# robotseu/ORB_Line_SLAM

Hardware: AMD Instinct MI355X
Metric: stereo frames/s extract+match (ORB+LBD), KITTI 1242x375 (higher is better)
Workload: dtype u8; 1 GPU; C3: 1242x375 stereo, 2000 ORB + 500 LBD per image, extract + stereo point/line match + f2f LBD match + SearchByBoW vs the previous frame (synthetic k=10 L=6 vocabulary, ComputeBoW included); parallelism=frame-sharded x1, distinct_pairs=512, order=shuffled, scene=default

## Files before the change

### orb_line_slam_amd/csrc/bow_match.hip

```cpp
#include "olf_internal.hpp"
#include "device_math.hpp"
#include "search_math.hpp"
#include "../../include/orbline.h"

namespace olf {

constexpr int BM_TH_LOW = 50;

__global__ __launch_bounds__(256) void k_bow_descend_nodes(const uint4* __restrict__ slotDesc, const int* __restrict__ childOff, const int* __restrict__ slotNode,
                                                           const double* __restrict__ nodeWeight, const uint4* __restrict__ desc, const int* __restrict__ counts,
                                                           int cap, int img_stride, int nid_level, int* __restrict__ nodeOut)
{
    const int f = blockIdx.y, i = blockIdx.x * 256 + threadIdx.x;
    if (i >= cap) return;
    int nid = -1;
    if (i < counts[(size_t)f * img_stride]) {
        const uint4* d = desc + 2 * ((size_t)f * img_stride * cap + i);
        const uint4 f0 = d[0], f1 = d[1];
        int node = 0, level = 0;
        int b = childOff[0], e = childOff[1];
        while (e > b) {
            ++level;
            int best = b, bd = 257;
            for (int s = b; s < e; ++s) {
                const uint4 c0 = slotDesc[2 * (size_t)s], c1 = slotDesc[2 * (size_t)s + 1];
                const int dd = ham256(f0, f1, c0, c1);
                if (dd < bd) { bd = dd; best = s; }
            }
            node = slotNode[best];
            if (level == nid_level) nid = node;
            b = childOff[node]; e = childOff[node + 1];
        }
        if (!(nodeWeight[node] > 0)) nid = -1;
        else if (nid < 0) nid = 0;
    }
    nodeOut[(size_t)f * cap + i] = nid;
}

__global__ __launch_bounds__(256) void k_bow_sort_nodes(const int* __restrict__ nodeIn, int cap, int P, unsigned long long* __restrict__ sorted, int* __restrict__ mOut)
{
    extern __shared__ unsigned long long s_key[];
    __shared__ int s_m;
    const int f = blockIdx.x;
    if (threadIdx.x == 0) s_m = 0;
    __syncthreads();
    int mine = 0;
    for (int i = threadIdx.x; i < P; i += 256) {
        const int nd = i < cap ? nodeIn[(size_t)f * cap + i] : -1;
        s_key[i] = nd >= 0 ? ((unsigned long long)nd << 16) | (unsigned)i : ~0ull;
        mine += nd >= 0;
    }
    if (mine) atomicAdd(&s_m, mine);
    __syncthreads();
    for (int k = 2; k <= P; k <<= 1)
        for (int j = k >> 1; j > 0; j >>= 1) {
            for (int t = threadIdx.x; t < P / 2; t += 256) {
                const int lo = ((t & ~(j - 1)) << 1) | (t & (j - 1)), hi = lo | j;
                const bool up = (lo & k) == 0;
                const unsigned long long a = s_key[lo], b = s_key[hi];
                if ((a > b) == up) { s_key[lo] = b; s_key[hi] = a; }
            }
            __syncthreads();
        }
    for (int i = threadIdx.x; i < cap; i += 256) sorted[(size_t)f * cap + i] = s_key[i];
    if (threadIdx.x == 0) mOut[f] = s_m;
}

constexpr int BM_WAVES = 8;

template <int FORM>
__device__ __forceinline__ void bow_node_walk(const unsigned long long* __restrict__ SK, int kb, int ke, const unsigned long long* __restrict__ SF, int fb, int fe,
                                              const uint4* __restrict__ dK, const uint4* __restrict__ dF, const olf_keypoint* __restrict__ kK,
                                              const olf_keypoint* __restrict__ kF, const uint8_t* __restrict__ validK, const uint8_t* __restrict__ badK,
                                              float nnratio, int checkOri, int lane, int* row, uint8_t* taken, uint8_t* binOf, int* hist, int* n)
{
    for (int q = kb; q < ke; ++q) {
        const int iKF = (int)(SK[q] & 0xffffu);
        if (validK && !validK[iKF]) continue;
        if (badK && badK[iKF]) continue;
        const uint4 a0 = dK[2 * (size_t)iKF], a1 = dK[2 * (size_t)iKF + 1];
        int b1 = 256, bi = -1, b2 = 256;
        for (int c0 = fb; c0 < fe; c0 += 64) {
            const bool on = c0 + lane < fe;
            const int iF = on ? (int)(SF[c0 + lane] & 0xffffu) : 0;
            int d = 0x7fff;
            if (on && (FORM == OLF_BOW_KF_FRAME ? row[iF] < 0 : taken[iF] == 0)) {
                const uint4 x0 = dF[2 * (size_t)iF], x1 = dF[2 * (size_t)iF + 1];
                d = ham256(a0, a1, x0, x1);
            }
            const int key = wave_min_i32((d << 6) | lane);
            const int c1 = key >> 6, cl = key & 63;
            const int d2 = wave_min_i32(lane == cl ? 0x7fff : d);
            if (c1 < 0x7fff) {
                const int ci = __builtin_amdgcn_readlane(iF, cl);
                if (c1 < b1) { b2 = min(b1, min(d2, 256)); b1 = c1; bi = ci; }
                else b2 = min(b2, c1);
            }
        }
        if ((FORM == OLF_BOW_KF_FRAME ? b1 <= BM_TH_LOW : b1 < BM_TH_LOW) && static_cast<float>(b1) < nnratio * static_cast<float>(b2)) {
            if (lane == 0) {
                const int at = FORM == OLF_BOW_KF_FRAME ? bi : iKF;
                if (FORM == OLF_BOW_KF_FRAME) row[bi] = iKF;
                else { row[iKF] = bi; taken[bi] = 1; }
                if (checkOri) {
                    int bin = rot_bin(kK[iKF].angle, kF[bi].angle);
                    bin = min(max(bin, 0), HISTO_LENGTH - 1);
                    binOf[at] = (uint8_t)bin;
                    atomicAdd(&hist[bin], 1);
                }
                atomicAdd(n, 1);
            }
            __builtin_amdgcn_wave_barrier();
        }
    }
}

__global__ __launch_bounds__(64 * BM_WAVES) void k_search_by_bow(const unsigned long long* __restrict__ sortedAll, const int* __restrict__ mAll, const olf_keypoint* __restrict__ kps,
                                                       const uint4* __restrict__ desc, const int* __restrict__ counts, int cap, int img_stride,
                                                       const uint8_t* __restrict__ mpValid, const uint8_t* __restrict__ mpBad, float nnratio, int checkOri,
                                                       int* __restrict__ matches, int* __restrict__ nmatches)
{
    extern __shared__ int s_mem[];
    __shared__ int s_hist[HISTO_LENGTH], s_seg, s_n, s_keep[3];
    int* matched = s_mem;
    uint8_t* binOf = reinterpret_cast<uint8_t*>(s_mem + cap);
    const int p = blockIdx.x, lane = threadIdx.x & 63;
    const int fK = p, fF = p + 1;
    const unsigned long long* SK = sortedAll + (size_t)fK * cap;
    const unsigned long long* SF = sortedAll + (size_t)fF * cap;
    const int mK = mAll[fK], mF = mAll[fF], nF = counts[(size_t)fF * img_stride];
    const olf_keypoint* kK = kps + (size_t)fK * img_stride * cap;
    const olf_keypoint* kF = kps + (size_t)fF * img_stride * cap;
    const uint4* dK = desc + 2 * (size_t)fK * img_stride * cap;
    const uint4* dF = desc + 2 * (size_t)fF * img_stride * cap;
    for (int i = threadIdx.x; i < cap; i += 64 * BM_WAVES) { matched[i] = -1; binOf[i] = 0; }
    if (threadIdx.x < HISTO_LENGTH) s_hist[threadIdx.x] = 0;
    if (threadIdx.x == 0) { s_seg = 0; s_n = 0; }
    __syncthreads();
    for (;;) {
        int kb = 0, ke = 0;
        if (lane == 0) {
            for (;;) {
                kb = atomicAdd(&s_seg, 0);
                if (kb >= mK) { ke = kb; break; }
                const unsigned long long node = SK[kb] >> 16;
                ke = bm_lower_bound(SK, mK, (node + 1) << 16);
                if (atomicCAS(&s_seg, kb, ke) == kb) break;
            }
        }
        kb = __builtin_amdgcn_readfirstlane(kb); ke = __builtin_amdgcn_readfirstlane(ke);
        if (kb >= mK) break;
        const unsigned long long node = SK[kb] >> 16;
        const int fb = bm_lower_bound(SF, mF, node << 16), fe = bm_lower_bound(SF, mF, (node + 1) << 16);
        if (fe <= fb) continue;
        bow_node_walk<OLF_BOW_KF_FRAME>(SK, kb, ke, SF, fb, fe, dK, dF, kK, kF, mpValid ? mpValid + (size_t)fK * cap : nullptr,
                                        mpBad ? mpBad + (size_t)fK * cap : nullptr, nnratio, checkOri, lane, matched, nullptr, binOf, s_hist, &s_n);
    }
    __syncthreads();
    if (checkOri) {
        if (threadIdx.x == 0) {
            int ind1, ind2, ind3;
            three_maxima(s_hist, ind1, ind2, ind3);
            s_keep[0] = ind1; s_keep[1] = ind2; s_keep[2] = ind3;
        }
        __syncthreads();
        int dropped = 0;
        for (int i = threadIdx.x; i < nF; i += 64 * BM_WAVES)
            if (matched[i] >= 0) { const int b = binOf[i]; if (b != s_keep[0] && b != s_keep[1] && b != s_keep[2]) { matched[i] = -1; ++dropped; } }
        if (dropped) atomicSub(&s_n, dropped);
        __syncthreads();
    }
    for (int i = threadIdx.x; i < cap; i += 64 * BM_WAVES) matches[(size_t)p * cap + i] = i < nF ? matched[i] : -1;
    if (threadIdx.x == 0) nmatches[p] = s_n;
}

int launch_bow_feature_vectors(const uint8_t* slotDesc, const int* childOff, const int* slotNode, const double* nodeWeight, int nid_level, int n_frames,
                               int img_stride, int cap, const uint8_t* d_desc, const int* d_counts, int* d_nodes, unsigned long long* d_sorted, int* d_m,
                               hipStream_t s)
{
    int P = 64;
    while (P < cap) P <<= 1;
    hipLaunchKernelGGL(k_bow_descend_nodes, dim3((cap + 255) / 256, n_frames), dim3(256), 0, s, reinterpret_cast<const uint4*>(slotDesc), childOff, slotNode,
                       nodeWeight, reinterpret_cast<const uint4*>(d_desc), d_counts, cap, img_stride, nid_level, d_nodes);
    hipLaunchKernelGGL(k_bow_sort_nodes, dim3(n_frames), dim3(256), (size_t)P * 8, s, d_nodes, cap, P, d_sorted, d_m);
    OLF_HIP_CHECK(hipGetLastError());
    return OLF_OK;
}

int launch_search_by_bow_batch(const uint8_t* slotDesc, const int* childOff, const int* slotNode, const double* nodeWeight, int nid_level, int n_frames,
                               int img_stride, int cap, const olf_keypoint* d_kps, const uint8_t* d_desc, const int* d_counts, const uint8_t* d_mp_valid,
                               const uint8_t* d_mp_bad, float nnratio, int check_ori, int* d_nodes, unsigned long long* d_sorted, int* d_m, int* d_matches,
                               int* d_nmatches, hipStream_t s)
{
    if (n_frames < 2) return OLF_OK;
    if (cap > 4096) { set_error("olf_search_by_bow_batch_dev: more than 4096 features per frame (the per-frame node sort runs in 32 KB of LDS)"); return OLF_ERR_CAPACITY; }
    OLF_TRY(launch_bow_feature_vectors(slotDesc, childOff, slotNode, nodeWeight, nid_level, n_frames, img_stride, cap, d_desc, d_counts, d_nodes, d_sorted, d_m, s));
    hipLaunchKernelGGL(k_search_by_bow, dim3(n_frames - 1), dim3(64 * BM_WAVES), (size_t)cap * 4 + ((cap + 3) & ~3), s, d_sorted, d_m, d_kps,
                       reinterpret_cast<const uint4*>(d_desc), d_counts, cap, img_stride, d_mp_valid, d_mp_bad, nnratio, check_ori, d_matches, d_nmatches);
    OLF_HIP_CHECK(hipGetLastError());
    return OLF_OK;
}

struct BowPairsArgs {
    const olf_keypoint* kps; const uint4* desc; const int* counts; const uint8_t* mpValid; const uint8_t* mpBad;
    const int* pairs;
    int cap, img_stride, n_frames, checkOri;
    float nnratio;
};

template <int FORM>
__global__ __launch_bounds__(64 * BM_WAVES) void k_search_by_bow_pairs(BowPairsArgs A, const unsigned long long* __restrict__ sortedAll, const int* __restrict__ mAll,
                                                                       int* __restrict__ status, int* __restrict__ matches, int* __restrict__ nmatches)
{
    extern __shared__ int s_mem[];
    __shared__ int s_hist[HISTO_LENGTH], s_seg, s_n, s_keep[3];
    const int cap = A.cap, p = blockIdx.x, tid = threadIdx.x, lane = tid & 63;
    int* row = s_mem;
    uint8_t* binOf = reinterpret_cast<uint8_t*>(s_mem + cap);
    uint8_t* taken = binOf + ((cap + 3) & ~3);
    const int f1 = A.pairs[2 * (size_t)p], f2 = A.pairs[2 * (size_t)p + 1];
    if (!pair_in_batch(f1, f2, A.n_frames)) {
        if (tid == 0) { nmatches[p] = -1; atomicOr(status, STATUS_PAIR); }
        return;
    }
    const size_t st = (size_t)A.img_stride;
    const unsigned long long* SK = sortedAll + (size_t)f1 * cap;
    const unsigned long long* SF = sortedAll + (size_t)f2 * cap;
    const int mK = mAll[f1], mF = mAll[f2];
    const int nRow = min(max(A.counts[(size_t)(FORM == OLF_BOW_KF_FRAME ? f2 : f1) * st], 0), cap);
    const olf_keypoint* kK = A.kps + (size_t)f1 * st * cap;
    const olf_keypoint* kF = A.kps + (size_t)f2 * st * cap;
    const uint4* dK = A.desc + 2 * (size_t)f1 * st * cap;
    const uint4* dF = A.desc + 2 * (size_t)f2 * st * cap;
    const uint8_t* validK = A.mpValid ? A.mpValid + (size_t)f1 * cap : nullptr;
    const uint8_t* badK = A.mpBad ? A.mpBad + (size_t)f1 * cap : nullptr;
    for (int i = tid; i < cap; i += 64 * BM_WAVES) {
        row[i] = -1; binOf[i] = 0;
        if (FORM == OLF_BOW_KF_KF) taken[i] = (A.mpValid && !A.mpValid[(size_t)f2 * cap + i]) || (A.mpBad && A.mpBad[(size_t)f2 * cap + i]) ? 1 : 0;
    }
    if (tid < HISTO_LENGTH) s_hist[tid] = 0;
    if (tid == 0) { s_seg = 0; s_n = 0; }
    __syncthreads();
    for (;;) {
        int kb = 0, ke = 0;
        if (lane == 0) {
            for (;;) {
                kb = atomicAdd(&s_seg, 0);
                if (kb >= mK) { ke = kb; break; }
                const unsigned long long node = SK[kb] >> 16;
                ke = bm_lower_bound(SK, mK, (node + 1) << 16);
                if (atomicCAS(&s_seg, kb, ke) == kb) break;
            }
        }
        kb = __builtin_amdgcn_readfirstlane(kb); ke = __builtin_amdgcn_readfirstlane(ke);
        if (kb >= mK) break;
        const unsigned long long node = SK[kb] >> 16;
        const int fb = bm_lower_bound(SF, mF, node << 16), fe = bm_lower_bound(SF, mF, (node + 1) << 16);
        if (fe <= fb) continue;
        bow_node_walk<FORM>(SK, kb, ke, SF, fb, fe, dK, dF, kK, kF, validK, badK, A.nnratio, A.checkOri, lane, row, taken, binOf, s_hist, &s_n);
    }
    __syncthreads();
    if (A.checkOri) {
        if (tid == 0) {
            int ind1, ind2, ind3;
            three_maxima(s_hist, ind1, ind2, ind3);
            s_keep[0] = ind1; s_keep[1] = ind2; s_keep[2] = ind3;
        }
        __syncthreads();
        int dropped = 0;
        for (int i = tid; i < nRow; i += 64 * BM_WAVES)
            if (row[i] >= 0) { const int b = binOf[i]; if (b != s_keep[0] && b != s_keep[1] && b != s_keep[2]) { row[i] = -1; ++dropped; } }
        if (dropped) atomicSub(&s_n, dropped);
        __syncthreads();
    }
    for (int i = tid; i < cap; i += 64 * BM_WAVES) matches[(size_t)p * cap + i] = row[i];
    if (tid == 0) nmatches[p] = s_n;
}

int launch_search_by_bow_pairs(const olf_track_batch& in, int n_frames, int cap, int n_pairs, const int* d_pairs, const uint8_t* d_mp_bad, int form, float nnratio,
                               int check_ori, const unsigned long long* d_sorted, const int* d_m, int* d_status, int* d_matches, int* d_nmatches, hipStream_t s)
{
    BowPairsArgs A;
    A.kps = in.kps; A.desc = reinterpret_cast<const uint4*>(in.desc); A.counts = in.counts; A.mpValid = in.mp_valid; A.mpBad = d_mp_bad;
    A.pairs = d_pairs; A.cap = cap; A.img_stride = in.img_stride; A.n_frames = n_frames; A.checkOri = check_ori; A.nnratio = nnratio;
    const size_t rowBytes = (size_t)cap * 4 + ((cap + 3) & ~3);
    if (form == OLF_BOW_KF_FRAME)
        hipLaunchKernelGGL(k_search_by_bow_pairs<OLF_BOW_KF_FRAME>, dim3(n_pairs), dim3(64 * BM_WAVES), rowBytes, s, A, d_sorted, d_m, d_status, d_matches, d_nmatches);
    else
        hipLaunchKernelGGL(k_search_by_bow_pairs<OLF_BOW_KF_KF>, dim3(n_pairs), dim3(64 * BM_WAVES), rowBytes + ((cap + 3) & ~3), s, A, d_sorted, d_m, d_status, d_matches,
                           d_nmatches);
    OLF_HIP_CHECK(hipGetLastError());
    return OLF_OK;
}

}
```

### orb_line_slam_amd/csrc/filters.hip

```cpp
#include "olf_internal.hpp"
#include <algorithm>

namespace olf {

constexpr int SF_TW = 128, SF_TH = 32;
constexpr int SF_INW = (SF_TW + 8) / 4;
constexpr int SF_INH = SF_TH + 6;

__device__ __forceinline__ int sf_reflect(int p, int n)
{
    if (p < 0) p = -p;
    if (p >= n) p = 2 * (n - 1) - p;
    return p;
}

__global__ __launch_bounds__(256) void k_sep7(const uint8_t* __restrict__ src, size_t srcImgStride, int srcPitch, uint8_t* __restrict__ dst,
                                              size_t dstImgStride, int dstPitch, int W, int H, Taps7 taps)
{
    __shared__ uint32_t s_in[SF_INH * SF_INW];
    constexpr int HS = (SF_INH + 1) / 2 + ((((SF_INH + 1) / 2) & 1) ? 0 : 1);
    __shared__ uint32_t s_h[SF_TW * HS];
    const int img = blockIdx.z, x0 = blockIdx.x * SF_TW, y0 = blockIdx.y * SF_TH;
    const uint8_t* s = src + (size_t)img * srcImgStride;
    const bool plain = x0 >= 4 && x0 + SF_TW + 4 <= W && y0 >= 3 && y0 + SF_TH + 3 <= H && ((srcPitch | (int)srcImgStride) & 3) == 0 &&
                       (reinterpret_cast<uintptr_t>(src) & 3) == 0;
    const uint8_t* tile = s + (ptrdiff_t)(y0 - 3) * srcPitch + (x0 - 4);
    for (int i = threadIdx.x; i < SF_INH * SF_INW; i += 256) {
        const int r = i / SF_INW, j = i - r * SF_INW;
        uint32_t v;
        if (plain) v = *reinterpret_cast<const uint32_t*>(tile + (size_t)r * srcPitch + 4 * j);
        else {
            const int gy = sf_reflect(min(y0 - 3 + r, H + 2), H);
            const int xw = x0 - 4 + 4 * j;
            const uint8_t* row = s + (size_t)gy * srcPitch;
            const uintptr_t addr = reinterpret_cast<uintptr_t>(row + xw);
            const int sh = (int)(addr & 3) * 8;
            if (xw >= 0 && (sh ? xw + 7 < W : xw + 3 < W)) {
                const uint32_t* p4 = reinterpret_cast<const uint32_t*>(row + xw - (int)(addr & 3));
                v = sh ? __funnelshift_r(p4[0], p4[1], sh) : p4[0];
            } else {
                v = 0;
#pragma unroll
                for (int b = 0; b < 4; ++b) v |= (uint32_t)row[sf_reflect(min(xw + b, W + 2), W)] << (8 * b);
            }
        }
        s_in[i] = v;
    }
    __syncthreads();
    const uint32_t tlo = (uint32_t)taps.t[0] | ((uint32_t)taps.t[1] << 8) | ((uint32_t)taps.t[2] << 16) | ((uint32_t)taps.t[3] << 24);
    const uint32_t thi = (uint32_t)taps.t[4] | ((uint32_t)taps.t[5] << 8) | ((uint32_t)taps.t[6] << 16);
    uint16_t* s_h16 = reinterpret_cast<uint16_t*>(s_h);
    for (int i = threadIdx.x; i < SF_INH * (SF_TW / 4); i += 256) {
        const int r = i / (SF_TW / 4), q = i - r * (SF_TW / 4);
        const uint32_t w0 = s_in[r * SF_INW + q], w1 = s_in[r * SF_INW + q + 1], w2 = s_in[r * SF_INW + q + 2];
        const uint32_t o0 = __builtin_amdgcn_udot4(__builtin_amdgcn_alignbyte(w2, w1, 1u), thi, __builtin_amdgcn_udot4(__builtin_amdgcn_alignbyte(w1, w0, 1u), tlo, 0u, false), false);
        const uint32_t o1 = __builtin_amdgcn_udot4(__builtin_amdgcn_alignbyte(w2, w1, 2u), thi, __builtin_amdgcn_udot4(__builtin_amdgcn_alignbyte(w1, w0, 2u), tlo, 0u, false), false);
        const uint32_t o2 = __builtin_amdgcn_udot4(__builtin_amdgcn_alignbyte(w2, w1, 3u), thi, __builtin_amdgcn_udot4(__builtin_amdgcn_alignbyte(w1, w0, 3u), tlo, 0u, false), false);
        const uint32_t o3 = __builtin_amdgcn_udot4(w2, thi, __builtin_amdgcn_udot4(w1, tlo, 0u, false), false);
        uint16_t* col = s_h16 + (size_t)(4 * q) * (2 * HS) + r;
        col[0] = (uint16_t)o0; col[2 * HS] = (uint16_t)o1; col[4 * HS] = (uint16_t)o2; col[6 * HS] = (uint16_t)o3;
    }
    __syncthreads();
    const int q = threadIdx.x & 31, ry0 = (threadIdx.x >> 5) * 4;
    const int gx = x0 + 4 * q;
    if (gx >= W) return;
    const uint32_t t01 = (uint32_t)taps.t[0] | ((uint32_t)taps.t[1] << 16), t23 = (uint32_t)taps.t[2] | ((uint32_t)taps.t[3] << 16);
    const uint32_t t45 = (uint32_t)taps.t[4] | ((uint32_t)taps.t[5] << 16), t6lo = (uint32_t)taps.t[6], t6hi = (uint32_t)taps.t[6] << 16;
    typedef unsigned short us2 __attribute__((ext_vector_type(2)));
    auto dot2 = [](uint32_t a, uint32_t b, uint32_t c) -> uint32_t {
        us2 va, vb;
        __builtin_memcpy(&va, &a, 4); __builtin_memcpy(&vb, &b, 4);
        return __builtin_amdgcn_udot2(va, vb, c, false);
    };
    uint32_t res[4][4];
#pragma unroll
    for (int c = 0; c < 4; ++c) {
        const uint32_t* hp = s_h + (size_t)(4 * q + c) * HS + (ry0 >> 1);
        const uint32_t D0 = hp[0], D1 = hp[1], D2 = hp[2], D3 = hp[3], D4 = hp[4];
        const uint32_t E0 = __builtin_amdgcn_alignbyte(D1, D0, 2u), E1 = __builtin_amdgcn_alignbyte(D2, D1, 2u);
        const uint32_t E2 = __builtin_amdgcn_alignbyte(D3, D2, 2u), E3 = __builtin_amdgcn_alignbyte(D4, D3, 2u);
        res[0][c] = dot2(D3, t6lo, dot2(D2, t45, dot2(D1, t23, dot2(D0, t01, 32768u))));
        res[1][c] = dot2(D3, t6hi, dot2(E2, t45, dot2(E1, t23, dot2(E0, t01, 32768u))));
        res[2][c] = dot2(D4, t6lo, dot2(D3, t45, dot2(D2, t23, dot2(D1, t01, 32768u))));
        res[3][c] = dot2(D4, t6hi, dot2(E3, t45, dot2(E2, t23, dot2(E1, t01, 32768u))));
    }
    uint8_t* d = dst + (size_t)img * dstImgStride;
#pragma unroll
    for (int rr = 0; rr < 4; ++rr) {
        const int gy = y0 + ry0 + rr;
        if (gy >= H) break;
        const uint32_t a0 = min(res[rr][0] >> 16, 255u), a1 = min(res[rr][1] >> 16, 255u), a2 = min(res[rr][2] >> 16, 255u), a3 = min(res[rr][3] >> 16, 255u);
        uint8_t* o = d + (size_t)gy * dstPitch + gx;
        if (gx + 3 < W && ((reinterpret_cast<uintptr_t>(o) & 3) == 0))
            *reinterpret_cast<uint32_t*>(o) = a0 | (a1 << 8) | (a2 << 16) | (a3 << 24);
        else {
            o[0] = (uint8_t)a0;
            if (gx + 1 < W) o[1] = (uint8_t)a1;
            if (gx + 2 < W) o[2] = (uint8_t)a2;
            if (gx + 3 < W) o[3] = (uint8_t)a3;
        }
    }
}

constexpr int SS_ROWS = 16;
constexpr int SS_BROWS = 8;

__device__ __forceinline__ int ss_reflect(int p, int n) { p = p < 0 ? -p : p; return p >= n ? 2 * (n - 1) - p : p; }

template <bool BORDER, int ROWS>
__device__ __forceinline__ void sep7_strip_body(const int t, const uint8_t* __restrict__ src, size_t srcImgStride, int srcPitch, uint8_t* __restrict__ dst,
                                                size_t dstImgStride, int dstPitch, int W, int H, const Taps7& taps, int nsx, int nsy)
{
    const int nb = BORDER ? 1 + ((W + 3) / 4 - (nsx + 1)) : nsx;
    if (t >= nb * nsy) return;
    const int sy = t / nb, si = t - sy * nb;
    const int sx = BORDER ? (si == 0 ? 0 : nsx + si) : si + 1;
    const int x0 = 4 * sx, y0 = sy * ROWS;
    const uint8_t* s = src + (size_t)blockIdx.y * srcImgStride + (x0 - 4);
    uint8_t* d = dst + (size_t)blockIdx.y * dstImgStride + x0;
    const uint32_t tlo = (uint32_t)taps.t[0] | ((uint32_t)taps.t[1] << 8) | ((uint32_t)taps.t[2] << 16) | ((uint32_t)taps.t[3] << 24);
    const uint32_t thi = (uint32_t)taps.t[4] | ((uint32_t)taps.t[5] << 8) | ((uint32_t)taps.t[6] << 16);
    const uint32_t t01 = (uint32_t)taps.t[0] | ((uint32_t)taps.t[1] << 16), t23 = (uint32_t)taps.t[2] | ((uint32_t)taps.t[3] << 16);
    const uint32_t t45 = (uint32_t)taps.t[4] | ((uint32_t)taps.t[5] << 16), t6lo = (uint32_t)taps.t[6], t6hi = (uint32_t)taps.t[6] << 16;
    typedef unsigned short us2 __attribute__((ext_vector_type(2)));
    auto dot2 = [](uint32_t a, uint32_t b, uint32_t c) -> uint32_t {
        us2 va, vb;
        __builtin_memcpy(&va, &a, 4); __builtin_memcpy(&vb, &b, 4);
        return __builtin_amdgcn_udot2(va, vb, c, false);
    };
    struct Raw { uint32_t w[3]; };
    auto load_row = [&](int y) -> Raw {
        Raw r;
        const uint8_t* row = s + (size_t)ss_reflect(min(y, H + 2), H) * srcPitch;
        if (!BORDER) __builtin_memcpy(r.w, row, 12);
        else {
#pragma unroll
            for (int k = 0; k < 3; ++k) {
                uint32_t v = 0;
#pragma unroll
                for (int b = 0; b < 4; ++b) {
                    const int x = x0 - 4 + 4 * k + b;
                    v |= (uint32_t)row[ss_reflect(min(x, W + 2), W) - (x0 - 4)] << (8 * b);
                }
                r.w[k] = v;
            }
        }
        return r;
    };
    auto hrow = [&](const Raw& r, uint32_t* o) {
        const uint32_t* w = r.w;
        o[0] = __builtin_amdgcn_udot4(__builtin_amdgcn_alignbyte(w[2], w[1], 1u), thi, __builtin_amdgcn_udot4(__builtin_amdgcn_alignbyte(w[1], w[0], 1u), tlo, 0u, false), false);
        o[1] = __builtin_amdgcn_udot4(__builtin_amdgcn_alignbyte(w[2], w[1], 2u), thi, __builtin_amdgcn_udot4(__builtin_amdgcn_alignbyte(w[1], w[0], 2u), tlo, 0u, false), false);
        o[2] = __builtin_amdgcn_udot4(__builtin_amdgcn_alignbyte(w[2], w[1], 3u), thi, __builtin_amdgcn_udot4(__builtin_amdgcn_alignbyte(w[1], w[0], 3u), tlo, 0u, false), false);
        o[3] = __builtin_amdgcn_udot4(w[2], thi, __builtin_amdgcn_udot4(w[1], tlo, 0u, false), false);
    };
    auto pair = [&](const Raw& ra, const Raw& rb, uint32_t* Pj) {
        uint32_t a[4], b[4];
        hrow(ra, a); hrow(rb, b);
#pragma unroll
        for (int c = 0; c < 4; ++c) Pj[c] = a[c] | (b[c] << 16);
    };
    uint32_t P[ROWS / 2 + 3][4];
    Raw nx[4];
    {
        Raw r0 = load_row(y0 - 3), r1 = load_row(y0 - 2), r2 = load_row(y0 - 1), r3 = load_row(y0), r4 = load_row(y0 + 1), r5 = load_row(y0 + 2);
#pragma unroll
        for (int k = 0; k < 4; ++k) nx[k] = load_row(y0 + 3 + k);
        pair(r0, r1, P[0]); pair(r2, r3, P[1]); pair(r4, r5, P[2]);
    }
#pragma unroll
    for (int g = 0; g < ROWS / 4; ++g) {
        const Raw c0 = nx[0], c1 = nx[1], c2 = nx[2], c3 = nx[3];
        if (g + 1 < ROWS / 4) {
#pragma unroll
            for (int k = 0; k < 4; ++k) nx[k] = load_row(y0 + 4 * (g + 1) + 3 + k);
            __builtin_amdgcn_sched_barrier(0);
        }
        pair(c0, c1, P[2 * g + 3]); pair(c2, c3, P[2 * g + 4]);
        uint32_t res[4][4];
#pragma unroll
        for (int c = 0; c < 4; ++c) {
            const uint32_t D0 = P[2 * g][c], D1 = P[2 * g + 1][c], D2 = P[2 * g + 2][c], D3 = P[2 * g + 3][c], D4 = P[2 * g + 4][c];
            const uint32_t E0 = __builtin_amdgcn_alignbyte(D1, D0, 2u), E1 = __builtin_amdgcn_alignbyte(D2, D1, 2u);
            const uint32_t E2 = __builtin_amdgcn_alignbyte(D3, D2, 2u), E3 = __builtin_amdgcn_alignbyte(D4, D3, 2u);
            res[0][c] = dot2(D3, t6lo, dot2(D2, t45, dot2(D1, t23, dot2(D0, t01, 32768u))));
            res[1][c] = dot2(D3, t6hi, dot2(E2, t45, dot2(E1, t23, dot2(E0, t01, 32768u))));
            res[2][c] = dot2(D4, t6lo, dot2(D3, t45, dot2(D2, t23, dot2(D1, t01, 32768u))));
            res[3][c] = dot2(D4, t6hi, dot2(E3, t45, dot2(E2, t23, dot2(E1, t01, 32768u))));
        }
#pragma unroll
        for (int rr = 0; rr < 4; ++rr) {
            const int gy = y0 + 4 * g + rr;
            if (gy < H) {
                const uint32_t a0 = min(res[rr][0] >> 16, 255u), a1 = min(res[rr][1] >> 16, 255u), a2 = min(res[rr][2] >> 16, 255u), a3 = min(res[rr][3] >> 16, 255u);
                const uint32_t v = a0 | (a1 << 8) | (a2 << 16) | (a3 << 24);
                if (!BORDER) __builtin_memcpy(d + (size_t)gy * dstPitch, &v, 4);
                else {
#pragma unroll
                    for (int b = 0; b < 4; ++b) if (x0 + b < W) d[(size_t)gy * dstPitch + b] = (uint8_t)(v >> (8 * b));
                }
            }
        }
    }
}

template <bool BORDER>
__global__ __launch_bounds__(256) void k_sep7_strip(const uint8_t* __restrict__ src, size_t srcImgStride, int srcPitch, uint8_t* __restrict__ dst,
                                                    size_t dstImgStride, int dstPitch, int W, int H, Taps7 taps, int nsx, int nsy)
{
    sep7_strip_body<BORDER, BORDER ? SS_BROWS : SS_ROWS>(blockIdx.x * 256 + threadIdx.x, src, srcImgStride, srcPitch, dst, dstImgStride, dstPitch, W, H, taps, nsx, nsy);
}

int launch_sep7(const uint8_t* src, size_t srcImgStride, int srcPitch, uint8_t* dst, size_t dstImgStride, int dstPitch, int W, int H,
                const int* taps7, int n_images, hipStream_t s)
{
    Taps7 t;
    for (int i = 0; i < 7; ++i) t.t[i] = taps7[i];
    if (t.t[3] == 256) {
        for (int i = 0; i < n_images; ++i)
            OLF_HIP_CHECK(hipMemcpy2DAsync(dst + (size_t)i * dstImgStride, dstPitch, src + (size_t)i * srcImgStride, srcPitch, W, H, hipMemcpyDeviceToDevice, s));
        return OLF_OK;
    }
    for (int i = 0; i < 7; ++i)
        if (t.t[i] < 0 || t.t[i] > 255) { set_error("launch_sep7: taps must be 8-bit fractions"); return OLF_ERR_INVALID; }
    if (W >= 16 && H >= 8 && (dstPitch & 3) == 0 && (dstImgStride & 3) == 0 && (reinterpret_cast<uintptr_t>(dst) & 3) == 0) {
        const int nsx = (W - 7) / 4, nsy = (H + SS_ROWS - 1) / SS_ROWS, nb = 1 + ((W + 3) / 4 - (nsx + 1));
        const int nsyB = (H + SS_BROWS - 1) / SS_BROWS;
        hipLaunchKernelGGL(k_sep7_strip<false>, dim3((nsx * nsy + 255) / 256, n_images), dim3(256), 0, s, src, srcImgStride, srcPitch, dst, dstImgStride, dstPitch, W, H, t, nsx, nsy);
        hipLaunchKernelGGL(k_sep7_strip<true>, dim3((nb * nsyB + 255) / 256, n_images), dim3(256), 0, s, src, srcImgStride, srcPitch, dst, dstImgStride, dstPitch, W, H, t, nsx, nsyB);
        OLF_HIP_CHECK(hipGetLastError());
        return OLF_OK;
    }
    hipLaunchKernelGGL(k_sep7, dim3((W + SF_TW - 1) / SF_TW, (H + SF_TH - 1) / SF_TH, n_images), dim3(256), 0, s, src, srcImgStride, srcPitch,
                       dst, dstImgStride, dstPitch, W, H, t);
    OLF_HIP_CHECK(hipGetLastError());
    return OLF_OK;
}

struct TapsWide { int r; int t[15]; };
__global__ __launch_bounds__(256) void k_sep_wide(const uint8_t* __restrict__ src, size_t srcImgStride, int srcPitch, uint8_t* __restrict__ dst,
                                                  size_t dstImgStride, int dstPitch, int W, int H, TapsWide taps)
{
    constexpr int TW = 64, TH = 16, RMAX = 7;
    __shared__ uint32_t s_h[TH + 2 * RMAX][TW];
    const int r = taps.r, n = 2 * r + 1;
    const int x0 = blockIdx.x * TW, y0 = blockIdx.y * TH;
    const uint8_t* in = src + (size_t)blockIdx.z * srcImgStride;
    uint8_t* out = dst + (size_t)blockIdx.z * dstImgStride;
    for (int i = threadIdx.x; i < (TH + 2 * r) * TW; i += 256) {
        const int ry = i / TW, cx = i - ry * TW, x = x0 + cx;
        int yy = y0 - r + ry;
        if (yy < 0) yy = -yy;
        if (yy >= H) yy = 2 * (H - 1) - yy;
        int acc = 0;
        if (x < W && yy >= 0 && yy < H) {
            const uint8_t* row = in + (size_t)yy * srcPitch;
            for (int k = 0; k < n; ++k) {
                int xx = x + k - r;
                if (xx < 0) xx = -xx;
                if (xx >= W) xx = 2 * (W - 1) - xx;
                acc += taps.t[k] * (int)row[xx];
            }
        }
        s_h[ry][cx] = (uint32_t)acc;
    }
    __syncthreads();
    for (int i = threadIdx.x; i < TH * TW; i += 256) {
        const int ty = i / TW, cx = i - ty * TW, x = x0 + cx, y = y0 + ty;
        if (x >= W || y >= H) continue;
        int acc = 0;
        for (int k = 0; k < n; ++k) acc += taps.t[k] * (int)s_h[ty + k][cx];
        const int v = (acc + 32768) >> 16;
        out[(size_t)y * dstPitch + x] = (uint8_t)(v > 255 ? 255 : v);
    }
}

int launch_sep_wide(const uint8_t* src, size_t srcImgStride, int srcPitch, uint8_t* dst, size_t dstImgStride, int dstPitch, int W, int H,
                    const int* taps, int r, int n_images, hipStream_t s)
{
    if (r < 1 || r > 7 || 2 * r >= W || 2 * r >= H) { set_error("launch_sep_wide: radius"); return OLF_ERR_INVALID; }
    TapsWide t; t.r = r;
    for (int i = 0; i < 15; ++i) t.t[i] = i < 2 * r + 1 ? taps[i] : 0;
    hipLaunchKernelGGL(k_sep_wide, dim3((W + 63) / 64, (H + 15) / 16, n_images), dim3(256), 0, s, src, srcImgStride, srcPitch, dst, dstImgStride,
                       dstPitch, W, H, t);
    OLF_HIP_CHECK(hipGetLastError());
    return OLF_OK;
}

constexpr int RZ_TW = 256, RZ_TH = 8, RZ_SW = 96 , RZ_SH = 16;

__global__ __launch_bounds__(256) void k_resize_tiled(const uint8_t* __restrict__ src, size_t srcImgStride, int srcPitch, int sw, int sh,
                                                      uint8_t* __restrict__ dst, size_t dstImgStride, int dstPitch, int dw, int dh,
                                                      const ResizeCoef* __restrict__ rx, const ResizeCoef* __restrict__ ry)
{
    __shared__ uint32_t s_src[RZ_SH * RZ_SW];
    __shared__ uint16_t s_h[RZ_SH * RZ_TW];
    __shared__ ResizeCoef s_rx[RZ_TW];
    const int img = blockIdx.z, dx0 = blockIdx.x * RZ_TW, dy0 = blockIdx.y * RZ_TH;
    const int nx = min(RZ_TW, dw - dx0), ny = min(RZ_TH, dh - dy0);
    const uint8_t* s = src + (size_t)img * srcImgStride;
    const int ry0 = min(max((int)ry[dy0].ofs, 0), sh - 1), ry1 = min(max((int)ry[dy0 + ny - 1].ofs + 1, 0), sh - 1);
    const int cx0 = ((int)rx[dx0].ofs) & ~3;
    const int cx1 = min((int)rx[dx0 + nx - 1].ofs + 1, sw - 1);
    const int nrows = ry1 - ry0 + 1, nwords = (cx1 - cx0) / 4 + 1;
    if (threadIdx.x < nx) s_rx[threadIdx.x] = rx[dx0 + threadIdx.x];
    for (int i = threadIdx.x; i < nrows * nwords; i += 256) {
        const int r = i / nwords, j = i - r * nwords;
        s_src[r * RZ_SW + j] = *reinterpret_cast<const uint32_t*>(s + (size_t)(ry0 + r) * srcPitch + cx0 + 4 * j);
    }
    __syncthreads();
    const uint8_t* sb = reinterpret_cast<const uint8_t*>(s_src);
    if ((int)threadIdx.x < nx) {
        const int x = threadIdx.x;
        const ResizeCoef c = s_rx[x];
        const int o0 = (int)c.ofs - cx0, o1 = min((int)c.ofs + 1, sw - 1) - cx0;
        const int a0 = c.a0, a1 = c.a1;
        for (int r = 0; r < nrows; ++r) {
            const int h = (int)sb[r * RZ_SW * 4 + o0] * a0 + (int)sb[r * RZ_SW * 4 + o1] * a1;
            s_h[r * RZ_TW + x] = (uint16_t)(h >> 4);
        }
    }
    __syncthreads();
    uint8_t* d = dst + (size_t)img * dstImgStride;
    for (int i = threadIdx.x; i < ny * (RZ_TW / 4); i += 256) {
        const int yy = i >> 6, q = i & 63;
        if (4 * q >= nx) continue;
        const ResizeCoef cy = ry[dy0 + yy];
        const int r0 = min(max((int)cy.ofs, 0), sh - 1) - ry0, r1 = min(max((int)cy.ofs + 1, 0), sh - 1) - ry0;
        const int b0 = cy.a0, b1 = cy.a1;
        uint32_t out = 0;
#pragma unroll
        for (int k = 0; k < 4; ++k) {
            const int h0 = s_h[r0 * RZ_TW + 4 * q + k], h1 = s_h[r1 * RZ_TW + 4 * q + k];
            const int v = (((b0 * h0) >> 16) + ((b1 * h1) >> 16) + 2) >> 2;
            out |= (uint32_t)(v & 0xff) << (8 * k);
        }
        *reinterpret_cast<uint32_t*>(d + (size_t)(dy0 + yy) * dstPitch + dx0 + 4 * q) = out;
    }
}

constexpr int RS_ROWS = 8;

__global__ __launch_bounds__(64) void k_resize_strip(const uint8_t* __restrict__ src, size_t srcImgStride, int srcPitch, int sw, int sh,
                                                     uint8_t* __restrict__ dst, size_t dstImgStride, int dstPitch, int dw, int dh,
                                                     const ResizeCoef* __restrict__ rx, const ResizeCoef* __restrict__ ry, int nsx)
{
    const int q = blockIdx.x * 64 + threadIdx.x;
    if (q >= nsx) return;
    const int dx0 = 4 * q, dy0 = blockIdx.y * RS_ROWS;
    const uint8_t* s = src + (size_t)blockIdx.z * srcImgStride;
    uint8_t* d = dst + (size_t)blockIdx.z * dstImgStride + dx0;
    typedef unsigned short us2 __attribute__((ext_vector_type(2)));
    uint32_t sel[4], coef[4];
    const int base = min((int)rx[dx0].ofs, srcPitch - 8);
#pragma unroll
    for (int k = 0; k < 4; ++k) {
        const ResizeCoef c = rx[min(dx0 + k, dw - 1)];
        const int o0 = (int)c.ofs - base, o1 = min((int)c.ofs + 1, sw - 1) - base;
        sel[k] = (uint32_t)o0 | 0x0c00u | ((uint32_t)o1 << 16) | 0x0c000000u;
        coef[k] = (uint32_t)(uint16_t)c.a0 | ((uint32_t)(uint16_t)c.a1 << 16);
    }
    struct Raw { uint32_t w[2]; };
    auto load_row = [&](int r) -> Raw { Raw v; __builtin_memcpy(v.w, s + (size_t)r * srcPitch + base, 8); return v; };
    auto hrow = [&](const Raw& v, uint32_t* h) {
#pragma unroll
        for (int k = 0; k < 4; ++k) {
            const uint32_t pr = __builtin_amdgcn_perm(v.w[1], v.w[0], sel[k]);
            us2 va, vb;
            __builtin_memcpy(&va, &pr, 4); __builtin_memcpy(&vb, &coef[k], 4);
            h[k] = __builtin_amdgcn_udot2(va, vb, 0u, false) >> 4;
        }
    };
    auto rows_of = [&](int dy, int& r0, int& r1, uint32_t& b0, uint32_t& b1) {
        const ResizeCoef cy = ry[min(dy, dh - 1)];
        r0 = min(max((int)cy.ofs, 0), sh - 1); r1 = min(max((int)cy.ofs + 1, 0), sh - 1);
        b0 = (uint32_t)cy.a0; b1 = (uint32_t)cy.a1;
    };
    int r0, r1, ra = -1, rb = -1;
    uint32_t b0, b1;
    rows_of(dy0, r0, r1, b0, b1);
    Raw p0 = load_row(r0), p1 = load_row(r1);
    uint32_t hA[4] = {0, 0, 0, 0}, hB[4] = {0, 0, 0, 0};
#pragma unroll
    for (int rr = 0; rr < RS_ROWS; ++rr) {
        const int dy = dy0 + rr;
        if (dy >= dh) break;
        int n0, n1;
        uint32_t c0, c1;
        rows_of(dy + 1, n0, n1, c0, c1);
        Raw q0 = p0, q1 = p1;
        if (rr + 1 < RS_ROWS) {
            if (n0 != r0 && n0 != r1) q0 = load_row(n0);
            if (n1 != n0 && n1 != r1) q1 = load_row(n1);
            __builtin_amdgcn_sched_barrier(0);
        }
        uint32_t h0[4], h1[4];
        if (r0 == ra) { for (int k = 0; k < 4; ++k) h0[k] = hA[k]; }
        else if (r0 == rb) { for (int k = 0; k < 4; ++k) h0[k] = hB[k]; }
        else hrow(p0, h0);
        if (r1 == r0) { for (int k = 0; k < 4; ++k) h1[k] = h0[k]; }
        else if (r1 == rb) { for (int k = 0; k < 4; ++k) h1[k] = hB[k]; }
        else hrow(p1, h1);
        uint32_t out = 0;
#pragma unroll
        for (int k = 0; k < 4; ++k) {
            const uint32_t v = (((b0 * h0[k]) >> 16) + ((b1 * h1[k]) >> 16) + 2u) >> 2;
            out |= (v & 0xffu) << (8 * k);
        }
        __builtin_memcpy(d + (size_t)dy * dstPitch, &out, 4);
        ra = r0; rb = r1;
#pragma unroll
        for (int k = 0; k < 4; ++k) { hA[k] = h0[k]; hB[k] = h1[k]; }
        r0 = n0; r1 = n1; b0 = c0; b1 = c1; p0 = q0; p1 = q1;
    }
}

bool resize_strip_fits(const ResizeCoef* rx, int sw, int dw, int ncols)
{
    for (int x0 = 0; x0 < dw; x0 += 4) {
        const int last = std::min(x0 + ncols - 1, dw - 1);
        if (std::min((int)rx[last].ofs + 1, sw - 1) - (int)rx[x0].ofs > 7) return false;
    }
    return sw >= 8;
}

bool resize_tiled_fits(const ResizeCoef* rx, const ResizeCoef* ry, int sw, int sh, int dw, int dh)
{
    for (int x0 = 0; x0 < dw; x0 += RZ_TW) {
        const int nx = std::min(RZ_TW, dw - x0);
        const int c0 = ((int)rx[x0].ofs) & ~3, c1 = std::min((int)rx[x0 + nx - 1].ofs + 1, sw - 1);
        if ((c1 - c0) / 4 + 1 > RZ_SW) return false;
    }
    for (int y0 = 0; y0 < dh; y0 += RZ_TH) {
        const int ny = std::min(RZ_TH, dh - y0);
        const int r0 = std::min(std::max((int)ry[y0].ofs, 0), sh - 1), r1 = std::min(std::max((int)ry[y0 + ny - 1].ofs + 1, 0), sh - 1);
        if (r1 - r0 + 1 > RZ_SH) return false;
    }
    return true;
}

int launch_resize_tiled(const uint8_t* src, size_t srcImgStride, int srcPitch, int sw, int sh, uint8_t* dst, size_t dstImgStride, int dstPitch,
                        int dw, int dh, const ResizeCoef* d_rx, const ResizeCoef* d_ry, int n_images, hipStream_t s, bool strip)
{
    strip = strip && (dstPitch & 3) == 0 && (dstImgStride & 3) == 0 && srcPitch >= 8;
    if (strip) {
        const int nsx = (dw + 3) / 4;
        hipLaunchKernelGGL(k_resize_strip, dim3((nsx + 63) / 64, (dh + RS_ROWS - 1) / RS_ROWS, n_images), dim3(64), 0, s, src, srcImgStride, srcPitch, sw, sh,
                           dst, dstImgStride, dstPitch, dw, dh, d_rx, d_ry, nsx);
        OLF_HIP_CHECK(hipGetLastError());
        return OLF_OK;
    }
    hipLaunchKernelGGL(k_resize_tiled, dim3((dw + RZ_TW - 1) / RZ_TW, (dh + RZ_TH - 1) / RZ_TH, n_images), dim3(256), 0, s, src, srcImgStride,
                       srcPitch, sw, sh, dst, dstImgStride, dstPitch, dw, dh, d_rx, d_ry);
    OLF_HIP_CHECK(hipGetLastError());
    return OLF_OK;
}

}
```

Baseline: 15040 stereo frames/s.

## Add single-chunk BoW walk fast path and rewrite sep7 border kernel

In the BoW node walk, when the frame-side node holds at most 64 features, each lane loads its frame descriptor once and reuses it across all keyframe features, with the next keyframe descriptor prefetched. This removes repeated descriptor loads and loop overhead in the common small-node case. Separately, the 7-tap filter's border kernel now fetches one aligned 12-byte window per row, rebuilds the reflected pixels with byte permutes, keeps a rolling vertical buffer, and launches 64-thread blocks instead of 256. The aim is to cut per-byte scattered loads on the image edges, at the cost of more register state and added code complexity.

```diff
diff --git a/orb_line_slam_amd/csrc/bow_match.hip b/orb_line_slam_amd/csrc/bow_match.hip
--- a/orb_line_slam_amd/csrc/bow_match.hip
+++ b/orb_line_slam_amd/csrc/bow_match.hip
@@ -74,6 +74,56 @@
                                               const olf_keypoint* __restrict__ kF, const uint8_t* __restrict__ validK, const uint8_t* __restrict__ badK,
                                               float nnratio, int checkOri, int lane, int* row, uint8_t* taken, uint8_t* binOf, int* hist, int* n)
 {
+    auto fold = [&](int d, int iF, int& b1, int& bi, int& b2) {
+        const int key = wave_min_i32((d << 6) | lane);
+        const int c1 = key >> 6, cl = key & 63;
+        const int d2 = wave_min_i32(lane == cl ? 0x7fff : d);
+        if (c1 < 0x7fff) {
+            const int ci = __builtin_amdgcn_readlane(iF, cl);
+            if (c1 < b1) { b2 = min(b1, min(d2, 256)); b1 = c1; bi = ci; }
+            else b2 = min(b2, c1);
+        }
+    };
+    auto accept = [&](int iKF, int b1, int bi, int b2) {
+        if ((FORM == OLF_BOW_KF_FRAME ? b1 <= BM_TH_LOW : b1 < BM_TH_LOW) && static_cast<float>(b1) < nnratio * static_cast<float>(b2)) {
+            if (lane == 0) {
+                const int at = FORM == OLF_BOW_KF_FRAME ? bi : iKF;
+                if (FORM == OLF_BOW_KF_FRAME) row[bi] = iKF;
+                else { row[iKF] = bi; taken[bi] = 1; }
+                if (checkOri) {
+                    int bin = rot_bin(kK[iKF].angle, kF[bi].angle);
+                    bin = min(max(bin, 0), HISTO_LENGTH - 1);
+                    binOf[at] = (uint8_t)bin;
+                    atomicAdd(&hist[bin], 1);
+                }
+                atomicAdd(n, 1);
+            }
+            __builtin_amdgcn_wave_barrier();
+        }
+    };
+    if (fe - fb <= 64) {
+        const bool on = fb + lane < fe;
+        const int iF = on ? (int)(SF[fb + lane] & 0xffffu) : 0;
+        uint4 x0 = make_uint4(0u, 0u, 0u, 0u), x1 = x0;
+        if (on) { x0 = dF[2 * (size_t)iF]; x1 = dF[2 * (size_t)iF + 1]; }
+        int iNext = (int)(SK[kb] & 0xffffu);
+        uint4 n0 = dK[2 * (size_t)iNext], n1 = dK[2 * (size_t)iNext + 1];
+        for (int q = kb; q < ke; ++q) {
+            const int iKF = iNext;
+            const uint4 a0 = n0, a1 = n1;
+            if (q + 1 < ke) {
+                iNext = (int)(SK[q + 1] & 0xffffu);
+                n0 = dK[2 * (size_t)iNext]; n1 = dK[2 * (size_t)iNext + 1];
+            }
+            if (validK && !validK[iKF]) continue;
+            if (badK && badK[iKF]) continue;
+            int b1 = 256, bi = -1, b2 = 256;
+            const int d = on && (FORM == OLF_BOW_KF_FRAME ? row[iF] < 0 : taken[iF] == 0) ? ham256(a0, a1, x0, x1) : 0x7fff;
+            fold(d, iF, b1, bi, b2);
+            accept(iKF, b1, bi, b2);
+        }
+        return;
+    }
     for (int q = kb; q < ke; ++q) {
         const int iKF = (int)(SK[q] & 0xffffu);
         if (validK && !validK[iKF]) continue;
@@ -88,30 +138,9 @@
                 const uint4 x0 = dF[2 * (size_t)iF], x1 = dF[2 * (size_t)iF + 1];
                 d = ham256(a0, a1, x0, x1);
             }
-            const int key = wave_min_i32((d << 6) | lane);
-            const int c1 = key >> 6, cl = key & 63;
-            const int d2 = wave_min_i32(lane == cl ? 0x7fff : d);
-            if (c1 < 0x7fff) {
-                const int ci = __builtin_amdgcn_readlane(iF, cl);
-                if (c1 < b1) { b2 = min(b1, min(d2, 256)); b1 = c1; bi = ci; }
-                else b2 = min(b2, c1);
-            }
-        }
-        if ((FORM == OLF_BOW_KF_FRAME ? b1 <= BM_TH_LOW : b1 < BM_TH_LOW) && static_cast<float>(b1) < nnratio * static_cast<float>(b2)) {
-            if (lane == 0) {
-                const int at = FORM == OLF_BOW_KF_FRAME ? bi : iKF;
-                if (FORM == OLF_BOW_KF_FRAME) row[bi] = iKF;
-                else { row[iKF] = bi; taken[bi] = 1; }
-                if (checkOri) {
-                    int bin = rot_bin(kK[iKF].angle, kF[bi].angle);
-                    bin = min(max(bin, 0), HISTO_LENGTH - 1);
-                    binOf[at] = (uint8_t)bin;
-                    atomicAdd(&hist[bin], 1);
-                }
-                atomicAdd(n, 1);
-            }
-            __builtin_amdgcn_wave_barrier();
-        }
+            fold(d, iF, b1, bi, b2);
+        }
+        accept(iKF, b1, bi, b2);
     }
 }
 
diff --git a/orb_line_slam_amd/csrc/filters.hip b/orb_line_slam_amd/csrc/filters.hip
--- a/orb_line_slam_amd/csrc/filters.hip
+++ b/orb_line_slam_amd/csrc/filters.hip
@@ -104,22 +104,33 @@
 
 constexpr int SS_ROWS = 16;
 constexpr int SS_BROWS = 8;
+constexpr int SS_BNT = 64;
 
 __device__ __forceinline__ int ss_reflect(int p, int n) { p = p < 0 ? -p : p; return p >= n ? 2 * (n - 1) - p : p; }
 
-template <bool BORDER, int ROWS>
+struct StripTaps {
+    uint32_t tlo, thi;
+    __device__ __forceinline__ explicit StripTaps(const Taps7& taps)
+        : tlo((uint32_t)taps.t[0] | ((uint32_t)taps.t[1] << 8) | ((uint32_t)taps.t[2] << 16) | ((uint32_t)taps.t[3] << 24)),
+          thi((uint32_t)taps.t[4] | ((uint32_t)taps.t[5] << 8) | ((uint32_t)taps.t[6] << 16)) {}
+    __device__ __forceinline__ void hrow(const uint32_t* w, uint32_t* o) const {
+        o[0] = __builtin_amdgcn_udot4(__builtin_amdgcn_alignbyte(w[2], w[1], 1u), thi, __builtin_amdgcn_udot4(__builtin_amdgcn_alignbyte(w[1], w[0], 1u), tlo, 0u, false), false);
+        o[1] = __builtin_amdgcn_udot4(__builtin_amdgcn_alignbyte(w[2], w[1], 2u), thi, __builtin_amdgcn_udot4(__builtin_amdgcn_alignbyte(w[1], w[0], 2u), tlo, 0u, false), false);
+        o[2] = __builtin_amdgcn_udot4(__builtin_amdgcn_alignbyte(w[2], w[1], 3u), thi, __builtin_amdgcn_udot4(__builtin_amdgcn_alignbyte(w[1], w[0], 3u), tlo, 0u, false), false);
+        o[3] = __builtin_amdgcn_udot4(w[2], thi, __builtin_amdgcn_udot4(w[1], tlo, 0u, false), false);
+    }
+};
+
+template <int ROWS>
 __device__ __forceinline__ void sep7_strip_body(const int t, const uint8_t* __restrict__ src, size_t srcImgStride, int srcPitch, uint8_t* __restrict__ dst,
                                                 size_t dstImgStride, int dstPitch, int W, int H, const Taps7& taps, int nsx, int nsy)
 {
-    const int nb = BORDER ? 1 + ((W + 3) / 4 - (nsx + 1)) : nsx;
-    if (t >= nb * nsy) return;
-    const int sy = t / nb, si = t - sy * nb;
-    const int sx = BORDER ? (si == 0 ? 0 : nsx + si) : si + 1;
+    if (t >= nsx * nsy) return;
+    const int sy = t / nsx, sx = t - sy * nsx + 1;
     const int x0 = 4 * sx, y0 = sy * ROWS;
     const uint8_t* s = src + (size_t)blockIdx.y * srcImgStride + (x0 - 4);
     uint8_t* d = dst + (size_t)blockIdx.y * dstImgStride + x0;
-    const uint32_t tlo = (uint32_t)taps.t[0] | ((uint32_t)taps.t[1] << 8) | ((uint32_t)taps.t[2] << 16) | ((uint32_t)taps.t[3] << 24);
-    const uint32_t thi = (uint32_t)taps.t[4] | ((uint32_t)taps.t[5] << 8) | ((uint32_t)taps.t[6] << 16);
+    const StripTaps st(taps);
     const uint32_t t01 = (uint32_t)taps.t[0] | ((uint32_t)taps.t[1] << 16), t23 = (uint32_t)taps.t[2] | ((uint32_t)taps.t[3] << 16);
     const uint32_t t45 = (uint32_t)taps.t[4] | ((uint32_t)taps.t[5] << 16), t6lo = (uint32_t)taps.t[6], t6hi = (uint32_t)taps.t[6] << 16;
     typedef unsigned short us2 __attribute__((ext_vector_type(2)));
@@ -131,32 +142,12 @@
     struct Raw { uint32_t w[3]; };
     auto load_row = [&](int y) -> Raw {
         Raw r;
-        const uint8_t* row = s + (size_t)ss_reflect(min(y, H + 2), H) * srcPitch;
-        if (!BORDER) __builtin_memcpy(r.w, row, 12);
-        else {
-#pragma unroll
-            for (int k = 0; k < 3; ++k) {
-                uint32_t v = 0;
-#pragma unroll
-                for (int b = 0; b < 4; ++b) {
-                    const int x = x0 - 4 + 4 * k + b;
-                    v |= (uint32_t)row[ss_reflect(min(x, W + 2), W) - (x0 - 4)] << (8 * b);
-                }
-                r.w[k] = v;
-            }
-        }
+        __builtin_memcpy(r.w, s + (size_t)ss_reflect(min(y, H + 2), H) * srcPitch, 12);
         return r;
-    };
-    auto hrow = [&](const Raw& r, uint32_t* o) {
-        const uint32_t* w = r.w;
-        o[0] = __builtin_amdgcn_udot4(__builtin_amdgcn_alignbyte(w[2], w[1], 1u), thi, __builtin_amdgcn_udot4(__builtin_amdgcn_alignbyte(w[1], w[0], 1u), tlo, 0u, false), false);
-        o[1] = __builtin_amdgcn_udot4(__builtin_amdgcn_alignbyte(w[2], w[1], 2u), thi, __builtin_amdgcn_udot4(__builtin_amdgcn_alignbyte(w[1], w[0], 2u), tlo, 0u, false), false);
-        o[2] = __builtin_amdgcn_udot4(__builtin_amdgcn_alignbyte(w[2], w[1], 3u), thi, __builtin_amdgcn_udot4(__builtin_amdgcn_alignbyte(w[1], w[0], 3u), tlo, 0u, false), false);
-        o[3] = __builtin_amdgcn_udot4(w[2], thi, __builtin_amdgcn_udot4(w[1], tlo, 0u, false), false);
     };
     auto pair = [&](const Raw& ra, const Raw& rb, uint32_t* Pj) {
         uint32_t a[4], b[4];
-        hrow(ra, a); hrow(rb, b);
+        st.hrow(ra.w, a); st.hrow(rb.w, b);
 #pragma unroll
         for (int c = 0; c < 4; ++c) Pj[c] = a[c] | (b[c] << 16);
     };
@@ -194,21 +185,66 @@
             if (gy < H) {
                 const uint32_t a0 = min(res[rr][0] >> 16, 255u), a1 = min(res[rr][1] >> 16, 255u), a2 = min(res[rr][2] >> 16, 255u), a3 = min(res[rr][3] >> 16, 255u);
                 const uint32_t v = a0 | (a1 << 8) | (a2 << 16) | (a3 << 24);
-                if (!BORDER) __builtin_memcpy(d + (size_t)gy * dstPitch, &v, 4);
-                else {
-#pragma unroll
-                    for (int b = 0; b < 4; ++b) if (x0 + b < W) d[(size_t)gy * dstPitch + b] = (uint8_t)(v >> (8 * b));
-                }
+                __builtin_memcpy(d + (size_t)gy * dstPitch, &v, 4);
             }
         }
     }
 }
 
+template <int ROWS>
+__device__ __forceinline__ void sep7_border_body(const int t, const uint8_t* __restrict__ src, size_t srcImgStride, int srcPitch, uint8_t* __restrict__ dst,
+                                                 size_t dstImgStride, int dstPitch, int W, int H, const Taps7& taps, int nsx, int nsy)
+{
+    const int nb = 1 + ((W + 3) / 4 - (nsx + 1));
+    if (t >= nb * nsy) return;
+    const int sy = t / nb, si = t - sy * nb;
+    const int sx = si == 0 ? 0 : nsx + si;
+    const int x0 = 4 * sx, y0 = sy * ROWS;
+    const uint8_t* s = src + (size_t)blockIdx.y * srcImgStride;
+    uint8_t* d = dst + (size_t)blockIdx.y * dstImgStride + x0;
+    const StripTaps st(taps);
+    int cb = W - 12;
+#pragma unroll
+    for (int k = 0; k < 12; ++k) cb = min(cb, ss_reflect(min(x0 - 4 + k, W + 2), W));
+    uint32_t selA[3] = {0u, 0u, 0u}, selB[3] = {0u, 0u, 0u};
+#pragma unroll
+    for (int k = 0; k < 12; ++k) {
+        const uint32_t si8 = (uint32_t)(ss_reflect(min(x0 - 4 + k, W + 2), W) - cb);
+        selA[k >> 2] |= (si8 < 8u ? si8 : 0x0cu) << (8 * (k & 3));
+        selB[k >> 2] |= (si8 < 8u ? 0x0cu : si8 - 8u) << (8 * (k & 3));
+    }
+    uint32_t h[7][4] = {};
+#pragma unroll 1
+    for (int y = y0 - 3; y < min(y0 + ROWS, H) + 3; ++y) {
+        uint32_t raw[3], w[3];
+        __builtin_memcpy(raw, s + (size_t)ss_reflect(y, H) * srcPitch + cb, 12);
+#pragma unroll
+        for (int k = 0; k < 3; ++k) w[k] = __builtin_amdgcn_perm(raw[1], raw[0], selA[k]) | __builtin_amdgcn_perm(raw[2], raw[2], selB[k]);
+#pragma unroll
+        for (int k = 0; k < 6; ++k)
+#pragma unroll
+            for (int c = 0; c < 4; ++c) h[k][c] = h[k + 1][c];
+        st.hrow(w, h[6]);
+        const int gy = y - 3;
+        if (gy >= y0) {
+#pragma unroll
+            for (int c = 0; c < 4; ++c) {
+                uint32_t acc = 32768u;
+#pragma unroll
+                for (int k = 0; k < 7; ++k) acc += h[k][c] * (uint32_t)taps.t[k];
+                if (x0 + c < W) d[(size_t)gy * dstPitch + c] = (uint8_t)min(acc >> 16, 255u);
+            }
+        }
+    }
+}
+
 template <bool BORDER>
-__global__ __launch_bounds__(256) void k_sep7_strip(const uint8_t* __restrict__ src, size_t srcImgStride, int srcPitch, uint8_t* __restrict__ dst,
-                                                    size_t dstImgStride, int dstPitch, int W, int H, Taps7 taps, int nsx, int nsy)
-{
-    sep7_strip_body<BORDER, BORDER ? SS_BROWS : SS_ROWS>(blockIdx.x * 256 + threadIdx.x, src, srcImgStride, srcPitch, dst, dstImgStride, dstPitch, W, H, taps, nsx, nsy);
+__global__ __launch_bounds__(BORDER ? SS_BNT : 256) __attribute__((amdgpu_waves_per_eu(BORDER ? 8 : 1, 8)))
+void k_sep7_strip(const uint8_t* __restrict__ src, size_t srcImgStride, int srcPitch, uint8_t* __restrict__ dst,
+                  size_t dstImgStride, int dstPitch, int W, int H, Taps7 taps, int nsx, int nsy)
+{
+    if (BORDER) sep7_border_body<SS_BROWS>(blockIdx.x * SS_BNT + threadIdx.x, src, srcImgStride, srcPitch, dst, dstImgStride, dstPitch, W, H, taps, nsx, nsy);
+    else sep7_strip_body<SS_ROWS>(blockIdx.x * 256 + threadIdx.x, src, srcImgStride, srcPitch, dst, dstImgStride, dstPitch, W, H, taps, nsx, nsy);
 }
 
 int launch_sep7(const uint8_t* src, size_t srcImgStride, int srcPitch, uint8_t* dst, size_t dstImgStride, int dstPitch, int W, int H,
@@ -227,7 +263,7 @@
         const int nsx = (W - 7) / 4, nsy = (H + SS_ROWS - 1) / SS_ROWS, nb = 1 + ((W + 3) / 4 - (nsx + 1));
         const int nsyB = (H + SS_BROWS - 1) / SS_BROWS;
         hipLaunchKernelGGL(k_sep7_strip<false>, dim3((nsx * nsy + 255) / 256, n_images), dim3(256), 0, s, src, srcImgStride, srcPitch, dst, dstImgStride, dstPitch, W, H, t, nsx, nsy);
-        hipLaunchKernelGGL(k_sep7_strip<true>, dim3((nb * nsyB + 255) / 256, n_images), dim3(256), 0, s, src, srcImgStride, srcPitch, dst, dstImgStride, dstPitch, W, H, t, nsx, nsyB);
+        hipLaunchKernelGGL(k_sep7_strip<true>, dim3((nb * nsyB + SS_BNT - 1) / SS_BNT, n_images), dim3(SS_BNT), 0, s, src, srcImgStride, srcPitch, dst, dstImgStride, dstPitch, W, H, t, nsx, nsyB);
         OLF_HIP_CHECK(hipGetLastError());
         return OLF_OK;
     }
```

Measured after the change: 15160 stereo frames/s (median of 6 runs). Within noise of the previous version (+0.8%).
